# NVIDIA-Merlin/Transformers4Rec

Hardware: AMD Instinct MI355X
Metric: training sessions/sec (XLNet 4x128, 100k items, seq 20, MLM, tied full softmax) + Recall@20 (higher is better)
Workload: dtype f32; 1 GPU; BASELINE.json configs[1]: synthetic schema, item vocab 100k (100001 table rows), d_model 128, 4-layer 4-head XLNet, seq_len 20, per-GPU batch 1024, MLM p=0.15, tied-weight full softmax, Adam, fwd+bwd+gradient exchange+optimizer per step; global_batch=1024, seq_len=20, parallelism=dp1, head_mode=materialize, precision_mode=auto, table_exchange=local, world_size=1, gpu_max_hw_queues=4, extra_streams=0, prefetch=1, preheat_steps=1695

## Files before the change

transformers4rec_amd/csrc/head_split.hip:

```cpp
#include "gemm_kernel.h"

namespace {

constexpr float kLog2e = 1.4426950408889634f;
typedef uint32_t u32x4 __attribute__((ext_vector_type(4)));
typedef float f32x4 __attribute__((ext_vector_type(4)));
__device__ __forceinline__ f32x16 mfma_bf16(u32x4 a, u32x4 b, f32x16 c) {
    return __builtin_amdgcn_mfma_f32_32x32x16_bf16(__builtin_bit_cast(bf16x8_t, a), __builtin_bit_cast(bf16x8_t, b), c, 0, 0, 0);
}

__device__ __forceinline__ void split8(const float (&x)[8], u32x4 (&w)[3]) {
    uint32_t a[3], b[3], c[3], d[3];
    cvt_pair<1>(x[0], x[1], a);
    cvt_pair<1>(x[2], x[3], b);
    cvt_pair<1>(x[4], x[5], c);
    cvt_pair<1>(x[6], x[7], d);
#pragma unroll
    for (int pl = 0; pl < 3; ++pl) w[pl] = u32x4{a[pl], b[pl], c[pl], d[pl]};
}
__device__ __forceinline__ f32x16 mfma6(const u32x4 (&a)[3], const u32x4 (&b)[3], f32x16 acc) {
    acc = mfma_bf16(a[1], b[1], acc);
    acc = mfma_bf16(a[2], b[0], acc);
    acc = mfma_bf16(a[0], b[2], acc);
    acc = mfma_bf16(a[1], b[0], acc);
// ... 380 lines not shown
            for (int i = 0; i < 4; ++i) {
                float x[4] = {v[i], v[4 + i], v[8 + i], v[12 + i]};
                quad_transpose4(x, t);
#pragma unroll
                for (int g = 0; g < 4; ++g) w[g][i] = x[g];
            }
            const int rq = b * 32 + (l32 & ~3);
            float* cq = C + (long)rq * ldc + vbase + 8 * t + 4 * khalf;
#pragma unroll
            for (int g = 0; g < 4; ++g)
                if (rq + g < N) {
                    const f32x4 o = {w[g][0], w[g][1], w[g][2], w[g][3]};
                    __builtin_nontemporal_store(o, reinterpret_cast<f32x4*>(cq + (long)g * ldc));
                }
        } else if (row < N) {
            float* cr = C + (long)row * ldc + c0;
#pragma unroll
            for (int r = 0; r < 16; ++r)
                if (c0 + 8 * (r >> 2) + (r & 3) < V) cr[8 * (r >> 2) + (r & 3)] = v[r];
        }
        float t = 0.f;
        if (tail_tile) {
#pragma unroll
            for (int r = 0; r < 16; ++r) {
                const bool in = c0 + 8 * (r >> 2) + (r & 3) < V;
                t += in ? v[r] : 0.f;
                v[r] = in ? v[r] : -INFINITY;
            }
        } else {
#pragma unroll
            for (int r = 0; r < 16; ++r) t += v[r];
        }
        float m = v[0];
#pragma unroll
        for (int r = 1; r < 16; ++r) m = fmaxf(m, v[r]);
        const float ref = (m == -INFINITY ? 0.f : m) * kLog2e;
        float se = 0.f;
#pragma unroll
        for (int r = 0; r < 16; ++r) se += __builtin_amdgcn_exp2f(fmaf(v[r], kLog2e, -ref));
        lse_merge(m, se, __shfl_xor(m, 32, 64), __shfl_xor(se, 32, 64));
        t += __shfl_xor(t, 32, 64);
        if (khalf == 0) sst[buf][wave][l32] = make_float4(m, se, t, 0.f);
        __syncthreads();
    }
    flush_stats((b_end - 1 - b_begin) & 1, b_end - 1);
    if (colmax) {
#pragma unroll
        for (int r = 0; r < 16; ++r) {
#pragma unroll
            for (int o = 16; o > 0; o >>= 1) cmax[r] = fmaxf(cmax[r], __shfl_xor(cmax[r], o, 64));
        }
        if (l32 == 0) {
            float* cp = colmax + (long)rsi * vpad + vbase + 4 * khalf;
#pragma unroll
            for (int g = 0; g < 4; ++g)
                *reinterpret_cast<float4*>(cp + 8 * g) = make_float4(cmax[4 * g], cmax[4 * g + 1], cmax[4 * g + 2], cmax[4 * g + 3]);
        }
    }
}

template <int NB, bool HS = false>
__global__ __launch_bounds__(256) void head_logits_ce_kernel(const u32x4* __restrict__ XA, const float* __restrict__ W,
                                                              long ldw, float* __restrict__ C, long ldc, int N, int V,
                                                              float alpha, int nblk, int blk_per, int vec_ok,
                                                              float* __restrict__ st_m, float* __restrict__ st_s,
                                                              float* __restrict__ st_t, int n_tile, int n_split,
                                                              const unsigned* __restrict__ amax = nullptr,
                                                              float* __restrict__ colmax = nullptr, int vpad = 0) {
    head_logits_ce_body<NB, false>(XA, W, ldw, C, ldc, N, V, alpha, nblk, blk_per, vec_ok, st_m, st_s, st_t, n_tile, n_split, amax,
                                   colmax, vpad);
}
template <int NB>
__global__ __launch_bounds__(256) __attribute__((amdgpu_waves_per_eu(3, 3))) void head_logits_ce_h_kernel(
    const u32x4* __restrict__ XA, const float* __restrict__ W, long ldw, float* __restrict__ C, long ldc, int N, int V, float alpha,
    int nblk, int blk_per, int vec_ok, float* __restrict__ st_m, float* __restrict__ st_s, float* __restrict__ st_t, int n_tile,
    int n_split, const unsigned* __restrict__ amax, float* __restrict__ colmax, int vpad) {
    head_logits_ce_body<NB, true>(XA, W, ldw, C, ldc, N, V, alpha, nblk, blk_per, vec_ok, st_m, st_s, st_t, n_tile, n_split, amax,
                                  colmax, vpad);
}
template <int NB>
__global__ __launch_bounds__(256) __attribute__((amdgpu_waves_per_eu(3, 3))) void head_ce_stats_h_kernel(
    const u32x4* __restrict__ XA, const float* __restrict__ W, long ldw, int N, int V, float alpha, int nblk, int blk_per,
    float* __restrict__ st_m, float* __restrict__ st_s, float* __restrict__ st_t, int n_tile, int n_split,
    const unsigned* __restrict__ amax, float* __restrict__ colmax, int vpad, const long* __restrict__ labels,
    float* __restrict__ zlab) {
    head_logits_ce_body<NB, true, true>(XA, W, ldw, nullptr, 0, N, V, alpha, nblk, blk_per, 1, st_m, st_s, st_t, n_tile, n_split, amax,
                                        colmax, vpad, labels, zlab);
}

__global__ __launch_bounds__(1024) void head_dw_aux_kernel(const float* __restrict__ lse, const long* __restrict__ labels, int N,
                                                            int yoff, int Vc, float* __restrict__ lse_min,
                                                            unsigned char* __restrict__ islab, int vpad) {
    __shared__ float red[16];
    for (int i = threadIdx.x; i < vpad / 16; i += 1024) reinterpret_cast<uint4*>(islab)[i] = make_uint4(0u, 0u, 0u, 0u);
    for (int i = (vpad / 16) * 16 + threadIdx.x; i < vpad; i += 1024) islab[i] = 0;
    __threadfence_block();
    __syncthreads();
    float m = INFINITY;
    for (int i = threadIdx.x; i < N; i += 1024) {
        m = fminf(m, lse[i]);
        const long y = labels[i] - yoff;
        if (y >= 0 && y < Vc) islab[y] = 1;
    }
#pragma unroll
    for (int o = 32; o > 0; o >>= 1) m = fminf(m, __shfl_xor(m, o, 64));
    if ((threadIdx.x & 63) == 0) red[threadIdx.x >> 6] = m;
    __syncthreads();
    if (threadIdx.x == 0) {
        for (int w = 1; w < 16; ++w) m = fminf(m, red[w]);
        *lse_min = fminf(m, red[0]);
    }
}

__global__ __launch_bounds__(1024) void head_ce_finalize_kernel(const float* __restrict__ st_m, const float* __restrict__ st_s,
                                                                 const float* __restrict__ st_t, int n_tiles, int N, int V,
                                                                 const float* __restrict__ C, long ldc,
                                                                 const long* __restrict__ labels, float smoothing,
                                                                 float* __restrict__ loss_rows, float* __restrict__ lse_out,
                                                                 const float* __restrict__ zlab = nullptr) {
    __shared__ float sm[32][33], ss[32][33], stt[32][33];
    const int r = threadIdx.x & 31, sl = threadIdx.x >> 5;
    const int row = min(blockIdx.x * 32 + r, N - 1);
    float m = -INFINITY, s = 0.f, t = 0.f;
    for (int k = sl; k < n_tiles; k += 32) {
        const long o = (long)k * N + row;
        lse_merge(m, s, st_m[o], st_s[o]);
        if (st_t) t += st_t[o];
    }
    sm[sl][r] = m; ss[sl][r] = s; stt[sl][r] = t;
    __syncthreads();
    if (sl == 0 && blockIdx.x * 32 + r < N) {
        for (int k = 1; k < 32; ++k) { lse_merge(m, s, sm[k][r], ss[k][r]); t += stt[k][r]; }
        const float lse = m + __logf(s);
        float loss = lse - (zlab ? zlab[row] : C[(long)row * ldc + labels[row]]);
        if (smoothing > 0.f) loss = (1.f - smoothing) * loss + smoothing * (lse - t / V);
        loss_rows[row] = loss;
        lse_out[row] = lse;
    }
}

struct SgScalars { float g, sub, hit; };
__device__ __forceinline__ float sg_value(float x, float l2, bool is_label, const SgScalars& q) {
    const float t = __builtin_amdgcn_exp2f(fmaf(x, kLog2e, -l2));
    return fmaf(q.g, t, -q.sub) - (is_label ? q.hit : 0.f);
}

struct DwAux { const float* colmax; const float* lse_min; const unsigned char* islab; int vpad, rsplit; };
__device__ __forceinline__ float pow2_scale_head(float m) {
    if (!(m > 0.f) || !(m < 3e38f)) return 1.f;
    int e;
    (void)frexpf(m, &e);
    return ldexpf(1.f, min(14 - e, 100));
}
template <int NB, bool HS = false, int PD = 1, bool NT = false, bool COPY = true, int WPS = 2>
__global__ __launch_bounds__(256, WPS) void head_dw_split_kernel(const float* __restrict__ logits, long ld,
                                                             const float* __restrict__ lse, const long* __restrict__ labels,
                                                             const float* __restrict__ gout, const u32x4* __restrict__ XT,
                                                             float* __restrict__ dW, long lddw, int N, int Vc, int V,
                                                             int yoff, float smooth, float alpha, int accumulate, int nblk,
                                                             const unsigned* __restrict__ amax = nullptr, DwAux dw = DwAux()) {
    constexpr int D = 32 * NB, NPL = HS ? 2 : 3;
    constexpr int BLK = 4 * NPL * 32 * NB;
    constexpr int SN = (BLK + 255) / 256;
    __shared__ u32x4 lds[2][BLK];
    __shared__ float2 rinfo[2][32];
    const int tid = threadIdx.x, lane = tid & 63, wave = tid >> 6, l32 = lane & 31, khalf = lane >> 5;
    const int v = blockIdx.x * 128 + 32 * wave + l32;
    const float* lp = logits + min(v, Vc - 1);
    SgScalars q;
    q.g = (gout ? *gout : 1.f) / N;
    __shared__ float sh_inv[4][32];
    if (HS) {
        float zmax = -INFINITY;
        for (int sidx = 0; sidx < dw.rsplit; ++sidx) zmax = fmaxf(zmax, dw.colmax[(long)sidx * dw.vpad + min(v, Vc - 1)]);
        const float pb = dw.islab[min(v, Vc - 1)] ? 1.f : __expf(fminf(zmax - *dw.lse_min, 0.f)) + smooth / V;
        const float bound = fabsf(q.g) * pb;
        const float sv = pow2_scale_head(bound);
        if (khalf == 0) sh_inv[wave][l32] = 1.f / sv;
        q.g *= sv;
        alpha = alpha / scale_of(amax);
    }
    q.sub = q.g * smooth / V;
    q.hit = q.g * (1.f - smooth);

    u32x4 st[SN];
    float ri_lse = 0.f;
    long ri_lab = 0;
    float xq[PD][16];
    auto g_load = [&](int b) __attribute__((always_inline)) {
        const u32x4* src = XT + (long)b * BLK;
#pragma unroll
        for (int i = 0; i < SN; ++i)
            if (BLK % 256 == 0 || i * 256 + tid < BLK) st[i] = src[i * 256 + tid];
        const int row = min(b * 32 + (tid & 31), N - 1);
        ri_lse = lse[row];
        ri_lab = labels[row];
    };
    auto x_load = [&](float (&x)[16], int b) __attribute__((always_inline)) {
        if (b * 32 + 32 <= N) {
            const float* base = lp + (long)(b * 32 + 8 * khalf) * ld;
#pragma unroll
            for (int s = 0; s < 2; ++s)
#pragma unroll
                for (int e = 0; e < 8; ++e) {
                    const float* a = base + (long)(16 * s + e) * ld;
                    x[8 * s + e] = NT ? __builtin_nontemporal_load(a) : *a;
                }
        } else {
#pragma unroll
            for (int s = 0; s < 2; ++s)
#pragma unroll
                for (int e = 0; e < 8; ++e) {
                    const float* a = lp + (long)min(b * 32 + 16 * s + 8 * khalf + e, N - 1) * ld;
                    x[8 * s + e] = NT ? __builtin_nontemporal_load(a) : *a;
                }
        }
    };
    auto s_store = [&](int buf, int b) __attribute__((always_inline)) {
#pragma unroll
        for (int i = 0; i < SN; ++i)
            if (BLK % 256 == 0 || i * 256 + tid < BLK) lds[buf][i * 256 + tid] = st[i];
        const bool live = b * 32 + (tid & 31) < N;
        if (tid < 32)
            rinfo[buf][tid] = live ? make_float2(ri_lse * kLog2e, __int_as_float((int)(ri_lab - yoff))) : make_float2(1e30f, __int_as_float(-1));
    };
    f32x16 acc[NB];
#pragma unroll
    for (int j = 0; j < NB; ++j)
#pragma unroll
        for (int r = 0; r < 16; ++r) acc[j][r] = 0.f;

    g_load(0);
#pragma unroll
    for (int u = 0; u < PD; ++u) x_load(xq[u], min(u, nblk - 1));
    s_store(0, 0);
    __syncthreads();
    for (int b0 = 0; b0 < nblk; b0 += PD) {
#pragma unroll
        for (int u = 0; u < PD; ++u) {
            const int b = b0 + u;
            if (b >= nblk) break;
            const int buf = b & 1;
            float xc[16];
#pragma unroll
            for (int i = 0; i < 16; ++i) xc[i] = xq[u][i];
            g_load(min(b + 1, nblk - 1));
            if (COPY) x_load(xq[u], min(b + PD, nblk - 1));
            __builtin_amdgcn_sched_barrier(0);
            u32x4 af[2][NPL];
#pragma unroll
            for (int s = 0; s < 2; ++s) {
                float gv[8];
#pragma unroll
                for (int e = 0; e < 8; ++e) {
                    const float2 in = rinfo[buf][16 * s + 8 * khalf + e];
                    gv[e] = sg_value(xc[8 * s + e], in.x, __float_as_int(in.y) == v, q);
                }
                split8s<HS>(gv, 1.f, af[s]);
            }
            if (!COPY) {
                __builtin_amdgcn_sched_barrier(0);
                x_load(xq[u], min(b + PD, nblk - 1));
                __builtin_amdgcn_sched_barrier(0);
            }
#pragma unroll
            for (int s = 0; s < 2; ++s)
#pragma unroll
                for (int j = 0; j < NB; ++j) {
                    u32x4 bf[NPL];
#pragma unroll
                    for (int pl = 0; pl < NPL; ++pl) bf[pl] = lds[buf][(pl * 4 + 2 * s + khalf) * D + 32 * j + l32];
                    acc[j] = mfma_split<HS>(af[s], bf, acc[j]);
                }
            s_store(buf ^ 1, min(b + 1, nblk - 1));
            __syncthreads();
        }
    }
    const int v0 = blockIdx.x * 128 + 32 * wave + 4 * khalf;
#pragma unroll
    for (int j = 0; j < NB; ++j) {
        float* cp = dW + (long)v0 * lddw + 32 * j + l32;
        float old[16];
        if (accumulate) {
#pragma unroll
            for (int r = 0; r < 16; ++r) old[r] = cp[(long)min((r & 3) + 8 * (r >> 2), Vc - 1 - v0) * lddw];
        }
#pragma unroll
        for (int r = 0; r < 16; ++r) {
            const int dr = (r & 3) + 8 * (r >> 2);
            const float a = HS ? alpha * sh_inv[wave][dr + 4 * khalf] : alpha;
            if (v0 + dr < Vc) cp[(long)dr * lddw] = a * acc[j][r] + (accumulate ? old[r] : 0.f);
        }
    }
}

template <int NB, bool HS = false>
__global__ __launch_bounds__(256) void head_dx_split_kernel(const float* __restrict__ logits, long ld,
                                                             const float* __restrict__ lse, const long* __restrict__ labels,
                                                             const float* __restrict__ gout, const u32x4* __restrict__ WT,
                                                             float* __restrict__ part, int N, int Vc, int V, int yoff,
                                                             float smooth, float alpha, int nkt, int kt_per, int row_tiles,
                                                             const unsigned* __restrict__ amax = nullptr) {
    constexpr int D = 32 * NB, NPL = HS ? 2 : 3;
    constexpr int BLK = 4 * NPL * 32 * NB;
    constexpr int SN = (BLK + 255) / 256;
    __shared__ u32x4 lds[2][BLK];
    const int tid = threadIdx.x, lane = tid & 63, wave = tid >> 6, l32 = lane & 31, khalf = lane >> 5;
    const int xcd = blockIdx.x & 7, slot = blockIdx.x >> 3;
    const int rt = slot % row_tiles, split = (slot / row_tiles) * 8 + xcd;
    const int kt_begin = split * kt_per, kt_end = min(nkt, kt_begin + kt_per);
    if (kt_begin >= kt_end) return;
    const int row = rt * 128 + 32 * wave + l32, rc = min(row, N - 1);
    const float* lp = logits + (long)rc * ld;
    const float l2 = lse[rc] * kLog2e;
    const int y = (int)(labels[rc] - yoff);
    SgScalars q;
    q.g = (gout ? *gout : 1.f) / N;
    if (HS) {
        int e;
        (void)frexpf(fabsf(q.g), &e);
        const float sg = (q.g != 0.f && fabsf(q.g) < 3e38f) ? ldexpf(1.f, min(14 - e, 100)) : 1.f;
        q.g *= sg;
        alpha = (alpha / sg) / scale_of(amax);
    }
    q.sub = q.g * smooth / V;
    q.hit = q.g * (1.f - smooth);
    const int ldm4 = (int)ld - 4;

    u32x4 st[SN];
    float4 xn[4];
    auto g_load = [&](int kt) __attribute__((always_inline)) {
        const u32x4* src = WT + (long)kt * BLK;
#pragma unroll
        for (int i = 0; i < SN; ++i)
            if (BLK % 256 == 0 || i * 256 + tid < BLK) st[i] = src[i * 256 + tid];
#pragma unroll
        for (int s = 0; s < 2; ++s) {
            const int c = kt * 32 + 16 * s + 8 * khalf;
            xn[2 * s] = *reinterpret_cast<const float4*>(lp + min(c, ldm4));
            xn[2 * s + 1] = *reinterpret_cast<const float4*>(lp + min(c + 4, ldm4));
        }
    };
    auto s_store = [&](int buf) __attribute__((always_inline)) {
#pragma unroll
        for (int i = 0; i < SN; ++i)
            if (BLK % 256 == 0 || i * 256 + tid < BLK) lds[buf][i * 256 + tid] = st[i];
    };
    f32x16 acc[NB];
#pragma unroll
    for (int j = 0; j < NB; ++j)
#pragma unroll
        for (int r = 0; r < 16; ++r) acc[j][r] = 0.f;

    g_load(kt_begin);
    s_store(0);
    __syncthreads();
    for (int kt = kt_begin; kt < kt_end; ++kt) {
        const int buf = (kt - kt_begin) & 1;
        float xc[16];
#pragma unroll
        for (int i = 0; i < 4; ++i) { xc[4 * i] = xn[i].x; xc[4 * i + 1] = xn[i].y; xc[4 * i + 2] = xn[i].z; xc[4 * i + 3] = xn[i].w; }
        g_load(min(kt + 1, kt_end - 1));
        __builtin_amdgcn_sched_barrier(0);
        if (kt * 32 + 32 > Vc) {
#pragma unroll
            for (int i = 0; i < 16; ++i)
                if (kt * 32 + 16 * (i >> 3) + 8 * khalf + (i & 7) >= Vc) xc[i] = -INFINITY;
        }
        u32x4 af[2][NPL];
#pragma unroll
        for (int s = 0; s < 2; ++s) {
            const int dy = y - (kt * 32 + 16 * s + 8 * khalf);
            float gv[8];
#pragma unroll
            for (int e = 0; e < 8; ++e) gv[e] = sg_value(xc[8 * s + e], l2, dy == e, q);
            split8s<HS>(gv, 1.f, af[s]);
        }
#pragma unroll
        for (int s = 0; s < 2; ++s)
#pragma unroll
            for (int j = 0; j < NB; ++j) {
                u32x4 bf[NPL];
#pragma unroll
                for (int pl = 0; pl < NPL; ++pl) bf[pl] = lds[buf][(pl * 4 + 2 * s + khalf) * D + 32 * j + l32];
                acc[j] = mfma_split<HS>(af[s], bf, acc[j]);
            }
        s_store(buf ^ 1);
        __syncthreads();
    }
    float* pp = part + (long)split * N * D;
    const int r0 = rt * 128 + 32 * wave + 4 * khalf;
#pragma unroll
    for (int j = 0; j < NB; ++j)
#pragma unroll
        for (int r = 0; r < 16; ++r) {
            const int rr = r0 + (r & 3) + 8 * (r >> 2);
            if (rr < N) pp[(long)rr * D + 32 * j + l32] = alpha * acc[j][r];
        }
}

template <int NB>
__global__ __launch_bounds__(256) void head_dw_rc_kernel(const u32x4* __restrict__ XA, const u32x4* __restrict__ XTP,
                                                          const float* __restrict__ W, long ldw, const float* __restrict__ lse,
                                                          const long* __restrict__ labels, const float* __restrict__ gout,
                                                          float* __restrict__ dW, long lddw, int N, int V, float smooth, float alpha,
                                                          int accumulate, int nblk, const unsigned* __restrict__ amax, DwAux dw) {
    constexpr int D = 32 * NB, KS = 2 * NB, CH = 4 * NB;
    constexpr int BLK = 4 * 2 * 32 * NB;
    constexpr int SN = (BLK + 255) / 256;
    __shared__ u32x4 ldsA[2][BLK];
    __shared__ u32x4 ldsT[2][BLK];
    __shared__ float2 rinfo[2][32];
    __shared__ float sh_inv[4][32];
    const int tid = threadIdx.x, lane = tid & 63, wave = tid >> 6, l32 = lane & 31, khalf = lane >> 5;
    const int v = blockIdx.x * 128 + 32 * wave + l32, vc = min(v, V - 1);
    const float sx = scale_of(amax), sw = scale_of(amax + 1);
    const float zscale = (alpha / sx) / sw;
    u32x4 Bf[KS][2];
    {
        const float* wr = W + (long)vc * ldw + 8 * khalf;
#pragma unroll
        for (int s = 0; s < KS; ++s) {
            const float4 u = *reinterpret_cast<const float4*>(wr + 16 * s);
            const float4 t = *reinterpret_cast<const float4*>(wr + 16 * s + 4);
            const float x[8] = {u.x, u.y, u.z, u.w, t.x, t.y, t.z, t.w};
            split8s<true>(x, sw, Bf[s]);
        }
    }
    SgScalars q;
// ... 565 lines not shown
    w.islab = w.colmax + (long)w.cmrows * w.vpad * 4;
    w.xtp = w.islab + ((w.vpad + 255) / 256) * 256;
    w.wa = w.xtp + w.nblk * blk;
    w.zlab = w.wa + ((head_recompute_on() || head_fdx_on()) ? w.nkt * blk : 0);
    w.total = w.zlab + (((long)N * 4 + 255) / 256) * 256;
    return w;
}
bool aligned16(const void* p) { return ((uintptr_t)p & 15) == 0; }

}

struct FwdNote { const float* W; const float* logits; int Vw, V, N, colmax, dw_form, cm_rows; };
static_assert(sizeof(FwdNote) <= 64, "t4r_head_note is 64 bytes");
static inline FwdNote* note_of(void* p) { return reinterpret_cast<FwdNote*>(p); }
extern "C" int t4r_head_note_dw_form(const void* note) { return note ? reinterpret_cast<const FwdNote*>(note)->dw_form : 0; }
static int head_w_amax(hipStream_t st, const float* W, long ldw, int V, int D, unsigned* out) {
    if (hipMemsetAsync(out, 0, 4, st) != hipSuccess) { t4r_set_error("head_split: memset failed"); return -1; }
    const long n4 = (long)V * (D / 4);
    hipLaunchKernelGGL(amax_kernel, dim3((unsigned)min(256L, (n4 + 1023) / 1024)), dim3(1024), 0, st, W, ldw, (long)V, D, out);
    return 0;
}

#define T4R_NB_SWITCH(D, CALL)                \
    switch ((D) / 32) {                       \
        case 1: { constexpr int NB = 1; CALL; } break; \
        case 2: { constexpr int NB = 2; CALL; } break; \
        case 3: { constexpr int NB = 3; CALL; } break; \
        default: { constexpr int NB = 4; CALL; } break; \
    }

extern "C" int t4r_head_split_supported(int D) { return D >= 32 && D <= 128 && D % 32 == 0; }
extern "C" int t4r_head_split_fwd_products(void) { return head_fwd_fp16x2() ? 3 : 6; }

extern "C" long t4r_head_split_ws_bytes(int N, int V, int D) {
    if (!t4r_head_split_supported(D) || N <= 0 || V <= 0) return 0;
    return head_ws(N, V, D).total;
}

extern "C" int t4r_head_split_prepare(void* stream, const float* X, long ldx, int N, int D, int V, void* ws) {
    if (N <= 0) return 0;
    T4R_CHECK_ARG(t4r_head_split_supported(D) && X && ws, "head_split_prepare: unsupported width or null pointer");
    T4R_CHECK_ARG(aligned16(X) && ldx % 4 == 0 && aligned16(ws), "head_split_prepare: X must be 16-byte aligned with a pitch multiple of 4");
    const HeadWs w = head_ws(N, V, D);
    hipStream_t st = (hipStream_t)stream;
    u32x4* xa = reinterpret_cast<u32x4*>((char*)ws + w.xa);
    u32x4* xt = reinterpret_cast<u32x4*>((char*)ws + w.xt);
    if (head_fwd_fp16x2()) {
        unsigned* amax = reinterpret_cast<unsigned*>((char*)ws + w.scales);
        if (hipMemsetAsync(amax, 0, 8, st) != hipSuccess) { t4r_set_error("head_split_prepare: memset failed"); return -1; }
        const long n4 = (long)N * (D / 4);
        hipLaunchKernelGGL(amax_kernel, dim3((unsigned)min(256L, (n4 + 255) / 256)), dim3(256), 0, st, X, ldx, (long)N, D, amax);
        if (head_dw_fp16x2()) {
            u32x4* xth = reinterpret_cast<u32x4*>((char*)ws + w.xth);
            T4R_NB_SWITCH(D, hipLaunchKernelGGL(split_x_images_kernel<NB>, dim3(w.nblk, 3), dim3(256), 0, st, X, ldx, N, xa, xt, xth, amax));
            T4R_LAUNCH_CHECK();
            return 0;
        }
        T4R_NB_SWITCH(D, hipLaunchKernelGGL((split_mk_kernel<NB, true>), dim3(w.nblk), dim3(256), 0, st, X, ldx, N, xa, amax));
    } else {
        T4R_NB_SWITCH(D, hipLaunchKernelGGL(split_mk_kernel<NB>, dim3(w.nblk), dim3(256), 0, st, X, ldx, N, xa));
    }
    T4R_NB_SWITCH(D, hipLaunchKernelGGL(split_km_kernel<NB>, dim3(w.nblk), dim3(256), 0, st, X, ldx, N, xt));
    T4R_LAUNCH_CHECK();
    return 0;
}

extern "C" int t4r_head_split_recompute_supported(int D);
extern "C" int t4r_head_split_prepare_rc(void* stream, const float* X, long ldx, int N, int D, int V, void* ws) {
    if (N <= 0) return 0;
    T4R_CHECK_ARG(t4r_head_split_recompute_supported(D) && X && ws, "head_split_prepare_rc: unsupported (the two-way fp16 forms must be on) or null pointer");
    T4R_CHECK_ARG(aligned16(X) && ldx % 4 == 0 && aligned16(ws), "head_split_prepare_rc: X must be 16-byte aligned with a pitch multiple of 4");
    const HeadWs w = head_ws(N, V, D);
    unsigned* amax = reinterpret_cast<unsigned*>((char*)ws + w.scales);
    u32x4* xtp = reinterpret_cast<u32x4*>((char*)ws + w.xtp);
    T4R_NB_SWITCH(D, hipLaunchKernelGGL((split_kmp_kernel<NB, true>), dim3(w.nblk), dim3(256), 0, (hipStream_t)stream, X, ldx, N, xtp, amax));
    T4R_LAUNCH_CHECK();
    return 0;
}

extern "C" int t4r_head_split_logits(void* stream, void* ws, const float* W, long ldw, float* C, long ldc, int N,
                                     int V, int D, float alpha, void* note) {
    if (N <= 0 || V <= 0) return 0;
    T4R_CHECK_ARG(t4r_head_split_supported(D) && W && C && ws, "head_split_logits: unsupported width or null pointer");
    T4R_CHECK_ARG(aligned16(W) && ldw % 4 == 0, "head_split_logits: W must be 16-byte aligned with a pitch multiple of 4");
    const HeadWs w = head_ws(N, V, D);
    static int per_env = -1;
    if (per_env < 0) { const char* e = t4r_exp_getenv("T4R_HEAD_ROWS_PER_WG"); per_env = e ? atoi(e) : 12; }
    const int blk_per = max(1, min(w.nblk, per_env));
    const int rs = (w.nblk + blk_per - 1) / blk_per;
    const u32x4* xa = reinterpret_cast<const u32x4*>((const char*)ws + w.xa);
    dim3 grid((V + 127) / 128, rs);
    if (head_fwd_fp16x2()) {
        unsigned* amax = reinterpret_cast<unsigned*>((char*)ws + w.scales);
        if (head_w_amax((hipStream_t)stream, W, ldw, V, D, amax + 1)) return -1;
        if (note) *note_of(note) = FwdNote{W, C, V, V, N, 0, 0, 0};
        T4R_NB_SWITCH(D, hipLaunchKernelGGL((head_logits_split_kernel<NB, true>), grid, dim3(256), 0, (hipStream_t)stream, xa, W,
                                            ldw, C, ldc, N, V, alpha, w.nblk, blk_per, amax));
    } else {
        T4R_NB_SWITCH(D, hipLaunchKernelGGL(head_logits_split_kernel<NB>, grid, dim3(256), 0, (hipStream_t)stream, xa, W, ldw, C,
                                            ldc, N, V, alpha, w.nblk, blk_per));
    }
    T4R_LAUNCH_CHECK();
    return 0;
}

int t4r_mean_launch(hipStream_t stream, const float* x, int n, float* out);
extern "C" int t4r_head_split_logits_ce(void* stream, void* ws, const float* W, long ldw, float* C, long ldc,
                                        const long* labels, float* loss_rows, float* lse, float* loss_mean, int N, int V,
                                        int D, float alpha, float label_smoothing, void* note) {
    hipStream_t st = (hipStream_t)stream;
    if (N <= 0 || V <= 0) return loss_mean ? t4r_mean_launch(st, loss_rows, 0, loss_mean) : 0;
    T4R_CHECK_ARG(t4r_head_split_supported(D) && W && C && ws && (!labels || (loss_rows && lse)), "head_split_logits_ce: unsupported width or null pointer");
    T4R_CHECK_ARG(aligned16(W) && ldw % 4 == 0, "head_split_logits_ce: W must be 16-byte aligned with a pitch multiple of 4");
    const HeadWs w = head_ws(N, V, D);
    static int per_env = -1;
    if (per_env < 0) { const char* e = t4r_exp_getenv("T4R_HEAD_ROWS_PER_WG"); per_env = e ? atoi(e) : 12; }
    const int blk_per = max(1, min(w.nblk, per_env));
    const int rs = (w.nblk + blk_per - 1) / blk_per;
    const u32x4* xa = reinterpret_cast<const u32x4*>((const char*)ws + w.xa);
    float* sm = reinterpret_cast<float*>((char*)ws + w.stats);
    float* ss = sm + (long)w.ntile * N;
    float* stt = label_smoothing > 0.f ? ss + (long)w.ntile * N : nullptr;
    const int vec_ok = aligned16(C) && ldc % 4 == 0;
    dim3 grid(8 * ((w.ntile + 7) / 8) * rs);
    if (head_fwd_fp16x2()) {
        unsigned* amax = reinterpret_cast<unsigned*>((char*)ws + w.scales);
        if (head_w_amax(st, W, ldw, V, D, amax + 1)) return -1;
        float* colmax = nullptr;
        if (head_dw_fp16x2() && rs == w.rsplit && vec_ok) colmax = reinterpret_cast<float*>((char*)ws + w.colmax);
        if (note) *note_of(note) = FwdNote{W, C, V, V, N, colmax != nullptr, 0, 0};
        T4R_NB_SWITCH(D, hipLaunchKernelGGL(head_logits_ce_h_kernel<NB>, grid, dim3(256), 0, st, xa, W, ldw, C, ldc, N, V,
                                            alpha, w.nblk, blk_per, vec_ok, sm, ss, stt, w.ntile, rs, amax, colmax, w.vpad));
    } else {
        T4R_NB_SWITCH(D, hipLaunchKernelGGL(head_logits_ce_kernel<NB>, grid, dim3(256), 0, st, xa, W, ldw, C, ldc, N, V, alpha,
                                            w.nblk, blk_per, vec_ok, sm, ss, stt, w.ntile, rs));
    }
    if (labels)
        hipLaunchKernelGGL(head_ce_finalize_kernel, dim3((N + 31) / 32), dim3(1024), 0, st, sm, ss, stt, w.ntile, N, V, C, ldc,
                           labels, label_smoothing, loss_rows, lse);
    T4R_LAUNCH_CHECK();
    return labels && loss_mean ? t4r_mean_launch(st, loss_rows, N, loss_mean) : 0;
}

extern "C" int t4r_head_split_dw(void* stream, void* ws, const float* logits, long ld, const float* lse,
                                 const long* labels, const float* grad_out, float label_smoothing, float* dW, long lddw,
                                 int N, int Vc, int V, int yoff, int D, float alpha, int accumulate, void* note_p) {
    if (N <= 0 || Vc <= 0) return 0;
    T4R_CHECK_ARG(t4r_head_split_supported(D) && logits && lse && labels && dW && ws, "head_split_dw: unsupported width or null pointer");
    const HeadWs w = head_ws(N, V, D);
    const u32x4* xt = reinterpret_cast<const u32x4*>((const char*)ws + w.xt);
    FwdNote* note = note_of(note_p);
    const bool have_cm = note && note->colmax && note->logits == logits && note->V == V && note->N == N && Vc == V && yoff == 0;
    if (note) note->dw_form = (head_fwd_fp16x2() && head_dw_fp16x2() && have_cm) ? 2 : 1;
    if (head_fwd_fp16x2() && head_dw_fp16x2() && have_cm) {
        hipStream_t st = (hipStream_t)stream;
        const unsigned* amax = reinterpret_cast<const unsigned*>((const char*)ws + w.scales);
        float* lse_min = reinterpret_cast<float*>(const_cast<char*>((const char*)ws) + w.scales) + 2;
        unsigned char* islab = reinterpret_cast<unsigned char*>(const_cast<char*>((const char*)ws) + w.islab);
        hipLaunchKernelGGL(head_dw_aux_kernel, dim3(1), dim3(1024), 0, st, lse, labels, N, yoff, Vc, lse_min, islab, w.vpad);
        DwAux aux{reinterpret_cast<const float*>((const char*)ws + w.colmax), lse_min, islab, w.vpad, note->cm_rows > 0 ? note->cm_rows : w.rsplit};
        const u32x4* xth = reinterpret_cast<const u32x4*>((const char*)ws + w.xth);
        T4R_NB_SWITCH(D, hipLaunchKernelGGL((head_dw_split_kernel<NB, true, 1, true>), dim3((Vc + 127) / 128), dim3(256), 0, st, logits,
                                            ld, lse, labels, grad_out, xth, dW, lddw, N, Vc, V, yoff, label_smoothing, alpha,
                                            accumulate, w.nblk, amax, aux));
    } else {
        T4R_NB_SWITCH(D, hipLaunchKernelGGL(head_dw_split_kernel<NB>, dim3((Vc + 127) / 128), dim3(256), 0, (hipStream_t)stream,
                                            logits, ld, lse, labels, grad_out, xt, dW, lddw, N, Vc, V, yoff, label_smoothing,
                                            alpha, accumulate, w.nblk));
    }
    T4R_LAUNCH_CHECK();
    return 0;
}

extern "C" int t4r_head_split_dx(void* stream, void* ws, const float* logits, long ld, const float* lse,
                                 const long* labels, const float* grad_out, float label_smoothing, const float* W, long ldw,
                                 float* dX, long lddx, int N, int Vc, int V, int yoff, int D, float alpha, int accumulate,
                                 void* note_p) {
    if (N <= 0 || Vc <= 0) return 0;
    T4R_CHECK_ARG(t4r_head_split_supported(D) && logits && lse && labels && dX && W && ws, "head_split_dx: unsupported width or null pointer");
    T4R_CHECK_ARG(aligned16(logits) && ld % 4 == 0 && ld >= 8 && aligned16(dX) && lddx % 4 == 0,
                  "head_split_dx: logits / dX must be 16-byte aligned with pitches multiple of 4");
    const HeadWs w = head_ws(N, V, D);
    hipStream_t st = (hipStream_t)stream;
    u32x4* wt = reinterpret_cast<u32x4*>((char*)ws + w.wt);
    float* part = reinterpret_cast<float*>((char*)ws + w.part);
    const int nkt = (Vc + 31) / 32, row_tiles = (N + 127) / 128;
    const bool hs = head_fwd_fp16x2();
    unsigned* amax = reinterpret_cast<unsigned*>((char*)ws + w.scales) + 1;
    if (hs) {
        FwdNote* note = note_of(note_p);
        const bool same = note && note->W == W && note->Vw == Vc;
        if (!same) {
            if (head_w_amax(st, W, ldw, Vc, D, amax)) return -1;
            if (note) { note->W = W; note->Vw = Vc; }
        }
        T4R_NB_SWITCH(D, hipLaunchKernelGGL((split_km_kernel<NB, true>), dim3(nkt), dim3(256), 0, st, W, ldw, Vc, wt, amax));
    } else {
        T4R_NB_SWITCH(D, hipLaunchKernelGGL(split_km_kernel<NB>, dim3(nkt), dim3(256), 0, st, W, ldw, Vc, wt));
    }
    const int target = head_dx_target();
    int splits = max(1, min(min(w.max_split, nkt / 8), target / row_tiles));
    const int kt_per = (nkt + splits - 1) / splits;
    splits = (nkt + kt_per - 1) / kt_per;
    if (hs) {
        T4R_NB_SWITCH(D, hipLaunchKernelGGL((head_dx_split_kernel<NB, true>), dim3(row_tiles * 8 * ((splits + 7) / 8)), dim3(256),
                                            0, st, logits, ld, lse, labels, grad_out, wt, part, N, Vc, V, yoff, label_smoothing,
                                            alpha, nkt, kt_per, row_tiles, amax));
    } else {
        T4R_NB_SWITCH(D, hipLaunchKernelGGL(head_dx_split_kernel<NB>, dim3(row_tiles * 8 * ((splits + 7) / 8)), dim3(256), 0, st,
                                            logits, ld, lse, labels, grad_out, wt, part, N, Vc, V, yoff, label_smoothing, alpha,
                                            nkt, kt_per, row_tiles));
    }
    const long nd4 = (long)N * D / 4;
    hipLaunchKernelGGL(head_dx_reduce_kernel, dim3((unsigned)((nd4 + 255) / 256)), dim3(256), 0, st, part, splits, nd4, D / 4,
                       dX, lddx, accumulate);
    T4R_LAUNCH_CHECK();
    return 0;
}

extern "C" int t4r_head_split_recompute_supported(int D) { return t4r_head_split_supported(D) && head_recompute_on(); }

extern "C" int t4r_head_split_ce(void* stream, void* ws, const float* W, long ldw, const long* labels, float* loss_rows,
                                 float* lse, float* loss_mean, int N, int V, int D, float alpha, float label_smoothing, void* note) {
    hipStream_t st = (hipStream_t)stream;
    if (N <= 0 || V <= 0) return loss_mean ? t4r_mean_launch(st, loss_rows, 0, loss_mean) : 0;
    T4R_CHECK_ARG(t4r_head_split_recompute_supported(D) && W && ws && labels && loss_rows && lse, "head_split_ce: unsupported (the two-way fp16 form must be on) or null pointer");
    T4R_CHECK_ARG(aligned16(W) && ldw % 4 == 0, "head_split_ce: W must be 16-byte aligned with a pitch multiple of 4");
    const HeadWs w = head_ws(N, V, D);
    const int blk_per = max(1, min(w.nblk, head_rows_per_wg()));
    const int rs = (w.nblk + blk_per - 1) / blk_per;
    T4R_CHECK_ARG(rs == w.rsplit, "head_split_ce: row split mismatch");
    const u32x4* xa = reinterpret_cast<const u32x4*>((const char*)ws + w.xa);
    float* sm = reinterpret_cast<float*>((char*)ws + w.stats);
    float* ss = sm + (long)w.ntile * N;
    float* stt = label_smoothing > 0.f ? ss + (long)w.ntile * N : nullptr;
    unsigned* amax = reinterpret_cast<unsigned*>((char*)ws + w.scales);
    float* colmax = reinterpret_cast<float*>((char*)ws + w.colmax);
    float* zlab = reinterpret_cast<float*>((char*)ws + w.zlab);
    if (head_w_amax(st, W, ldw, V, D, amax + 1)) return -1;
    if (note) *note_of(note) = FwdNote{W, nullptr, V, V, N, 1, 0, 0};
    dim3 grid(8 * ((w.ntile + 7) / 8) * rs);
    T4R_NB_SWITCH(D, hipLaunchKernelGGL(head_ce_stats_h_kernel<NB>, grid, dim3(256), 0, st, xa, W, ldw, N, V, alpha, w.nblk, blk_per, sm, ss,
                                        stt, w.ntile, rs, amax, colmax, w.vpad, labels, zlab));
    hipLaunchKernelGGL(head_ce_finalize_kernel, dim3((N + 31) / 32), dim3(1024), 0, st, sm, ss, stt, w.ntile, N, V, (const float*)nullptr,
                       0L, labels, label_smoothing, loss_rows, lse, (const float*)zlab);
    T4R_LAUNCH_CHECK();
    return loss_mean ? t4r_mean_launch(st, loss_rows, N, loss_mean) : 0;
}

extern "C" int t4r_head_split_dw_rc(void* stream, void* ws, const float* W, long ldw, const float* lse, const long* labels,
                                    const float* grad_out, float label_smoothing, float* dW, long lddw, int N, int V, int D,
                                    float alpha, int accumulate, void* note_p) {
    if (N <= 0 || V <= 0) return 0;
    T4R_CHECK_ARG(t4r_head_split_recompute_supported(D) && W && lse && labels && dW && ws, "head_split_dw_rc: unsupported or null pointer");
    FwdNote* note = note_of(note_p);
    T4R_CHECK_ARG(note && note->colmax && note->W == W && note->V == V && note->N == N, "head_split_dw_rc: the note of this workspace's t4r_head_split_ce is required");
    const HeadWs w = head_ws(N, V, D);
    hipStream_t st = (hipStream_t)stream;
    const unsigned* amax = reinterpret_cast<const unsigned*>((const char*)ws + w.scales);
    float* lse_min = reinterpret_cast<float*>((char*)ws + w.scales) + 2;
    unsigned char* islab = reinterpret_cast<unsigned char*>((char*)ws + w.islab);
    hipLaunchKernelGGL(head_dw_aux_kernel, dim3(1), dim3(1024), 0, st, lse, labels, N, 0, V, lse_min, islab, w.vpad);
    DwAux aux{reinterpret_cast<const float*>((const char*)ws + w.colmax), lse_min, islab, w.vpad, w.rsplit};
    const u32x4* xa = reinterpret_cast<const u32x4*>((const char*)ws + w.xa);
    const u32x4* xtp = reinterpret_cast<const u32x4*>((const char*)ws + w.xtp);
    note->dw_form = 3;
    T4R_NB_SWITCH(D, hipLaunchKernelGGL(head_dw_rc_kernel<NB>, dim3((V + 127) / 128), dim3(256), 0, st, xa, xtp, W, ldw, lse, labels,
                                        grad_out, dW, lddw, N, V, label_smoothing, alpha, accumulate, w.nblk, amax, aux));
    T4R_LAUNCH_CHECK();
    return 0;
}

extern "C" int t4r_head_split_dx_rc(void* stream, void* ws, const float* X, long ldx, const float* W, long ldw, const float* lse,
                                    const long* labels, const float* grad_out, float label_smoothing, float* dX, long lddx,
                                    int N, int V, int D, float alpha, int accumulate, void* note_p) {
    if (N <= 0 || V <= 0) return 0;
    T4R_CHECK_ARG(t4r_head_split_recompute_supported(D) && X && W && lse && labels && dX && ws, "head_split_dx_rc: unsupported or null pointer");
    T4R_CHECK_ARG(aligned16(X) && ldx % 4 == 0 && aligned16(W) && ldw % 4 == 0 && aligned16(dX) && lddx % 4 == 0,
                  "head_split_dx_rc: X / W / dX must be 16-byte aligned with pitches multiple of 4");
    FwdNote* note = note_of(note_p);
    T4R_CHECK_ARG(note && note->W == W && note->Vw == V && note->N == N, "head_split_dx_rc: the note of this workspace's t4r_head_split_ce is required");
    const HeadWs w = head_ws(N, V, D);
    hipStream_t st = (hipStream_t)stream;
    const unsigned* amax = reinterpret_cast<const unsigned*>((const char*)ws + w.scales);
    u32x4* wtp = reinterpret_cast<u32x4*>((char*)ws + w.wt);
    u32x4* wa = reinterpret_cast<u32x4*>((char*)ws + w.wa);
    float* part = reinterpret_cast<float*>((char*)ws + w.part);
    const int nkt = w.nkt, row_tiles = (N + 127) / 128;
    T4R_NB_SWITCH(D, hipLaunchKernelGGL((split_mk_kernel<NB, true>), dim3(nkt), dim3(256), 0, st, W, ldw, V, wa, amax + 1));
    T4R_NB_SWITCH(D, hipLaunchKernelGGL((split_kmp_kernel<NB, true>), dim3(nkt), dim3(256), 0, st, W, ldw, V, wtp, amax + 1));
    const int target = head_dx_target();
    int splits = max(1, min(min(w.max_split, nkt / 8), target / row_tiles));
    const int kt_per = (nkt + splits - 1) / splits;
    splits = (nkt + kt_per - 1) / kt_per;
    T4R_NB_SWITCH(D, hipLaunchKernelGGL(head_dx_rc_kernel<NB>, dim3(row_tiles * 8 * ((splits + 7) / 8)), dim3(256), 0, st, X, ldx, wa, wtp,
                                        lse, labels, grad_out, part, N, V, label_smoothing, alpha, nkt, kt_per, row_tiles, amax));
    const long nd4 = (long)N * D / 4;
    hipLaunchKernelGGL(head_dx_reduce_kernel, dim3((unsigned)((nd4 + 255) / 256)), dim3(256), 0, st, part, splits, nd4, D / 4, dX, lddx,
                       accumulate);
    T4R_LAUNCH_CHECK();
    return 0;
}

static thread_local const float* g_w_amax_part = nullptr;
static thread_local const float* g_w_amax_W = nullptr;
static thread_local int g_w_amax_n = 0;
extern "C" void t4r_head_split_w_amax_hint(const float* W, const float* part, int n) {
    g_w_amax_W = (part && n > 0) ? W : nullptr; g_w_amax_part = g_w_amax_W ? part : nullptr; g_w_amax_n = g_w_amax_W ? n : 0;
}
extern "C" int t4r_head_split_fdx_supported(int D) { return t4r_head_split_supported(D) && head_fdx_on(); }
extern "C" int t4r_head_split_logits_ce_dx(void* stream, void* ws, const float* X, long ldx, const float* W, long ldw, float* C,
                                           long ldc, const long* labels, float* loss_rows, float* lse, float* loss_mean,
                                           float* dX, long lddx, const float* wsum, int N, int V, int D, float alpha,
                                           float label_smoothing, void* note) {
    hipStream_t st = (hipStream_t)stream;
    if (N <= 0 || V <= 0) return loss_mean ? t4r_mean_launch(st, loss_rows, 0, loss_mean) : 0;
    const bool kernel_only = labels == nullptr;
    T4R_CHECK_ARG(t4r_head_split_fdx_supported(D) && X && W && C && ws && (kernel_only || (loss_rows && lse && dX)),
                  "head_split_logits_ce_dx: unsupported (the two-way fp16 form must be on) or null pointer");
    T4R_CHECK_ARG(aligned16(X) && ldx % 4 == 0 && aligned16(W) && ldw % 4 == 0 && aligned16(dX) && lddx % 4 == 0,
                  "head_split_logits_ce_dx: X / W / dX must be 16-byte aligned with pitches multiple of 4");
// ... 40 lines not shown
```

Measured before the change: 400,700 sessions/s.

## Use buffer loads, ballot-gated label hits and vector LDS reads in head dW kernel

Restructures the tied-head dW split kernel. Logit tiles are now read with raw buffer loads using 32-bit offsets and a cache-policy bit, and the label-hit correction is skipped unless a wave ballot finds a label in its column range. Row LSE values are read from LDS as float4 vectors, labels are loaded as 32-bit ints, and the PD/COPY prefetch template knobs are removed. For D=128 the launch adds 24 KB of dynamic shared memory, apparently to limit occupancy, and a WIDE fallback path handles very large pitches.

```diff
diff --git a/transformers4rec_amd/csrc/head_split.hip b/transformers4rec_amd/csrc/head_split.hip
--- a/transformers4rec_amd/csrc/head_split.hip
+++ b/transformers4rec_amd/csrc/head_split.hip
@@ -556,8 +556,8 @@
     (void)frexpf(m, &e);
     return ldexpf(1.f, min(14 - e, 100));
 }
-template <int NB, bool HS = false, int PD = 1, bool NT = false, bool COPY = true, int WPS = 2>
-__global__ __launch_bounds__(256, WPS) void head_dw_split_kernel(const float* __restrict__ logits, long ld,
+template <int NB, bool HS = false, bool WIDE = false>
+__global__ __launch_bounds__(256, 2) void head_dw_split_kernel(const float* __restrict__ logits, long ld,
                                                              const float* __restrict__ lse, const long* __restrict__ labels,
                                                              const float* __restrict__ gout, const u32x4* __restrict__ XT,
                                                              float* __restrict__ dW, long lddw, int N, int Vc, int V,
@@ -566,18 +566,21 @@
     constexpr int D = 32 * NB, NPL = HS ? 2 : 3;
     constexpr int BLK = 4 * NPL * 32 * NB;
     constexpr int SN = (BLK + 255) / 256;
+    constexpr int POLICY = HS ? 2 : 0;
     __shared__ u32x4 lds[2][BLK];
-    __shared__ float2 rinfo[2][32];
+    __shared__ __attribute__((aligned(16))) float rinfo[2][32];
     const int tid = threadIdx.x, lane = tid & 63, wave = tid >> 6, l32 = lane & 31, khalf = lane >> 5;
     const int v = blockIdx.x * 128 + 32 * wave + l32;
-    const float* lp = logits + min(v, Vc - 1);
+    const int vc = min(v, Vc - 1);
+    const int ldb = WIDE ? 0 : (int)ld * 4;
+    const int voff = vc * 4 + 8 * khalf * ldb;
     SgScalars q;
     q.g = (gout ? *gout : 1.f) / N;
     __shared__ float sh_inv[4][32];
     if (HS) {
         float zmax = -INFINITY;
-        for (int sidx = 0; sidx < dw.rsplit; ++sidx) zmax = fmaxf(zmax, dw.colmax[(long)sidx * dw.vpad + min(v, Vc - 1)]);
-        const float pb = dw.islab[min(v, Vc - 1)] ? 1.f : __expf(fminf(zmax - *dw.lse_min, 0.f)) + smooth / V;
+        for (int sidx = 0; sidx < dw.rsplit; ++sidx) zmax = fmaxf(zmax, dw.colmax[(long)sidx * dw.vpad + vc]);
+        const float pb = dw.islab[vc] ? 1.f : __expf(fminf(zmax - *dw.lse_min, 0.f)) + smooth / V;
         const float bound = fabsf(q.g) * pb;
         const float sv = pow2_scale_head(bound);
         if (khalf == 0) sh_inv[wave][l32] = 1.f / sv;
@@ -589,8 +592,8 @@
 
     u32x4 st[SN];
     float ri_lse = 0.f;
-    long ri_lab = 0;
-    float xq[PD][16];
+    int ri_lab = 0;
+    float xq[16];
     auto g_load = [&](int b) __attribute__((always_inline)) {
         const u32x4* src = XT + (long)b * BLK;
 #pragma unroll
@@ -598,35 +601,40 @@
             if (BLK % 256 == 0 || i * 256 + tid < BLK) st[i] = src[i * 256 + tid];
         const int row = min(b * 32 + (tid & 31), N - 1);
         ri_lse = lse[row];
-        ri_lab = labels[row];
+        ri_lab = reinterpret_cast<const int*>(labels)[2 * row];
     };
     auto x_load = [&](float (&x)[16], int b) __attribute__((always_inline)) {
-        if (b * 32 + 32 <= N) {
-            const float* base = lp + (long)(b * 32 + 8 * khalf) * ld;
+        if constexpr (!WIDE) {
+            const int rows = min(32, N - 32 * b);
+            const auto rsrc = __builtin_amdgcn_make_buffer_rsrc(const_cast<float*>(logits + (long)b * 32 * ld), 0,
+                                                                ((rows - 1) * (int)ld + Vc) * 4, 0x00020000);
 #pragma unroll
             for (int s = 0; s < 2; ++s)
 #pragma unroll
-                for (int e = 0; e < 8; ++e) {
-                    const float* a = base + (long)(16 * s + e) * ld;
-                    x[8 * s + e] = NT ? __builtin_nontemporal_load(a) : *a;
-                }
+                for (int e = 0; e < 8; ++e)
+                    x[8 * s + e] = __uint_as_float(__builtin_amdgcn_raw_buffer_load_b32(rsrc, voff, (16 * s + e) * ldb, POLICY));
         } else {
+            const float* lp = logits + vc;
 #pragma unroll
             for (int s = 0; s < 2; ++s)
 #pragma unroll
                 for (int e = 0; e < 8; ++e) {
                     const float* a = lp + (long)min(b * 32 + 16 * s + 8 * khalf + e, N - 1) * ld;
-                    x[8 * s + e] = NT ? __builtin_nontemporal_load(a) : *a;
+                    x[8 * s + e] = POLICY ? __builtin_nontemporal_load(a) : *a;
                 }
         }
     };
+    const int wbase = blockIdx.x * 128 + 32 * wave;
+    int ylab = -1;
+    unsigned long hits = 0;
     auto s_store = [&](int buf, int b) __attribute__((always_inline)) {
 #pragma unroll
         for (int i = 0; i < SN; ++i)
             if (BLK % 256 == 0 || i * 256 + tid < BLK) lds[buf][i * 256 + tid] = st[i];
         const bool live = b * 32 + (tid & 31) < N;
-        if (tid < 32)
-            rinfo[buf][tid] = live ? make_float2(ri_lse * kLog2e, __int_as_float((int)(ri_lab - yoff))) : make_float2(1e30f, __int_as_float(-1));
+        rinfo[buf][tid & 31] = live ? ri_lse * kLog2e : 1e30f;
+        ylab = live ? ri_lab - yoff : -1;
+        hits = __builtin_amdgcn_ballot_w64((unsigned)(ylab - wbase) < 32u);
     };
     f32x16 acc[NB];
 #pragma unroll
@@ -635,50 +643,50 @@
         for (int r = 0; r < 16; ++r) acc[j][r] = 0.f;
 
     g_load(0);
-#pragma unroll
-    for (int u = 0; u < PD; ++u) x_load(xq[u], min(u, nblk - 1));
+    x_load(xq, 0);
     s_store(0, 0);
     __syncthreads();
-    for (int b0 = 0; b0 < nblk; b0 += PD) {
-#pragma unroll
-        for (int u = 0; u < PD; ++u) {
-            const int b = b0 + u;
-            if (b >= nblk) break;
-            const int buf = b & 1;
-            float xc[16];
-#pragma unroll
-            for (int i = 0; i < 16; ++i) xc[i] = xq[u][i];
-            g_load(min(b + 1, nblk - 1));
-            if (COPY) x_load(xq[u], min(b + PD, nblk - 1));
-            __builtin_amdgcn_sched_barrier(0);
-            u32x4 af[2][NPL];
-#pragma unroll
-            for (int s = 0; s < 2; ++s) {
-                float gv[8];
+    for (int b = 0; b < nblk; ++b) {
+        const int buf = b & 1;
+        g_load(min(b + 1, nblk - 1));
+        __builtin_amdgcn_sched_barrier(0);
+        float gv[2][8];
+#pragma unroll
+        for (int s = 0; s < 2; ++s) {
+            const f32x4* rp = reinterpret_cast<const f32x4*>(&rinfo[buf][16 * s + 8 * khalf]);
+            const f32x4 la = rp[0], lb = rp[1];
+#pragma unroll
+            for (int e = 0; e < 8; ++e) {
+                const float t = __builtin_amdgcn_exp2f(fmaf(xq[8 * s + e], kLog2e, -(e < 4 ? la[e] : lb[e - 4])));
+                gv[s][e] = fmaf(q.g, t, -q.sub);
+            }
+        }
+        if (hits != 0) {
+#pragma unroll
+            for (int s = 0; s < 2; ++s)
 #pragma unroll
                 for (int e = 0; e < 8; ++e) {
-                    const float2 in = rinfo[buf][16 * s + 8 * khalf + e];
-                    gv[e] = sg_value(xc[8 * s + e], in.x, __float_as_int(in.y) == v, q);
+                    const int y0 = __builtin_amdgcn_readlane(ylab, 16 * s + e), y1 = __builtin_amdgcn_readlane(ylab, 16 * s + 8 + e);
+                    gv[s][e] -= (khalf ? y1 : y0) == v ? q.hit : 0.f;
                 }
-                split8s<HS>(gv, 1.f, af[s]);
+        }
+        __builtin_amdgcn_sched_barrier(0);
+        x_load(xq, min(b + 1, nblk - 1));
+        __builtin_amdgcn_sched_barrier(0);
+        u32x4 af[2][NPL];
+#pragma unroll
+        for (int s = 0; s < 2; ++s) split8s<HS>(gv[s], 1.f, af[s]);
+#pragma unroll
+        for (int s = 0; s < 2; ++s)
+#pragma unroll
+            for (int j = 0; j < NB; ++j) {
+                u32x4 bf[NPL];
+#pragma unroll
+                for (int pl = 0; pl < NPL; ++pl) bf[pl] = lds[buf][(pl * 4 + 2 * s + khalf) * D + 32 * j + l32];
+                acc[j] = mfma_split<HS>(af[s], bf, acc[j]);
             }
-            if (!COPY) {
-                __builtin_amdgcn_sched_barrier(0);
-                x_load(xq[u], min(b + PD, nblk - 1));
-                __builtin_amdgcn_sched_barrier(0);
-            }
-#pragma unroll
-            for (int s = 0; s < 2; ++s)
-#pragma unroll
-                for (int j = 0; j < NB; ++j) {
-                    u32x4 bf[NPL];
-#pragma unroll
-                    for (int pl = 0; pl < NPL; ++pl) bf[pl] = lds[buf][(pl * 4 + 2 * s + khalf) * D + 32 * j + l32];
-                    acc[j] = mfma_split<HS>(af[s], bf, acc[j]);
-                }
-            s_store(buf ^ 1, min(b + 1, nblk - 1));
-            __syncthreads();
-        }
+        s_store(buf ^ 1, min(b + 1, nblk - 1));
+        __syncthreads();
     }
     const int v0 = blockIdx.x * 128 + 32 * wave + 4 * khalf;
 #pragma unroll
@@ -1550,6 +1558,8 @@
     FwdNote* note = note_of(note_p);
     const bool have_cm = note && note->colmax && note->logits == logits && note->V == V && note->N == N && Vc == V && yoff == 0;
     if (note) note->dw_form = (head_fwd_fp16x2() && head_dw_fp16x2() && have_cm) ? 2 : 1;
+    const bool wide = ld >= (1L << 24);
+    const dim3 grid((Vc + 127) / 128);
     if (head_fwd_fp16x2() && head_dw_fp16x2() && have_cm) {
         hipStream_t st = (hipStream_t)stream;
         const unsigned* amax = reinterpret_cast<const unsigned*>((const char*)ws + w.scales);
@@ -1558,13 +1568,23 @@
         hipLaunchKernelGGL(head_dw_aux_kernel, dim3(1), dim3(1024), 0, st, lse, labels, N, yoff, Vc, lse_min, islab, w.vpad);
         DwAux aux{reinterpret_cast<const float*>((const char*)ws + w.colmax), lse_min, islab, w.vpad, note->cm_rows > 0 ? note->cm_rows : w.rsplit};
         const u32x4* xth = reinterpret_cast<const u32x4*>((const char*)ws + w.xth);
-        T4R_NB_SWITCH(D, hipLaunchKernelGGL((head_dw_split_kernel<NB, true, 1, true>), dim3((Vc + 127) / 128), dim3(256), 0, st, logits,
-                                            ld, lse, labels, grad_out, xth, dW, lddw, N, Vc, V, yoff, label_smoothing, alpha,
-                                            accumulate, w.nblk, amax, aux));
+        if (wide) {
+            T4R_NB_SWITCH(D, hipLaunchKernelGGL((head_dw_split_kernel<NB, true, true>), grid, dim3(256), 0, st, logits, ld, lse, labels,
+                                                grad_out, xth, dW, lddw, N, Vc, V, yoff, label_smoothing, alpha, accumulate, w.nblk,
+                                                amax, aux));
+        } else {
+            const unsigned hold = D == 128 ? 24576 : 0;
+            T4R_NB_SWITCH(D, hipLaunchKernelGGL((head_dw_split_kernel<NB, true>), grid, dim3(256), hold, st, logits, ld, lse, labels,
+                                                grad_out, xth, dW, lddw, N, Vc, V, yoff, label_smoothing, alpha, accumulate, w.nblk,
+                                                amax, aux));
+        }
+    } else if (wide) {
+        T4R_NB_SWITCH(D, hipLaunchKernelGGL((head_dw_split_kernel<NB, false, true>), grid, dim3(256), 0, (hipStream_t)stream, logits, ld,
+                                            lse, labels, grad_out, xt, dW, lddw, N, Vc, V, yoff, label_smoothing, alpha, accumulate,
+                                            w.nblk));
     } else {
-        T4R_NB_SWITCH(D, hipLaunchKernelGGL(head_dw_split_kernel<NB>, dim3((Vc + 127) / 128), dim3(256), 0, (hipStream_t)stream,
-                                            logits, ld, lse, labels, grad_out, xt, dW, lddw, N, Vc, V, yoff, label_smoothing,
-                                            alpha, accumulate, w.nblk));
+        T4R_NB_SWITCH(D, hipLaunchKernelGGL(head_dw_split_kernel<NB>, grid, dim3(256), 0, (hipStream_t)stream, logits, ld, lse, labels,
+                                            grad_out, xt, dW, lddw, N, Vc, V, yoff, label_smoothing, alpha, accumulate, w.nblk));
     }
     T4R_LAUNCH_CHECK();
     return 0;
```

New measurement: 404,300 sessions/s (median of 4 runs). No clear change (+0.9%).
